# dpryan79/MethylDackel

Hardware: AMD Instinct MI355X
Metric: CpG calls/sec, synthetic 1 Mb contig 30x paired-end WGBS BAM, CpG extract (higher is better)
Workload: dtype u8/u32

## Files before the change

methyldackel_amd/csrc/mdk_prep.hip:

```cpp
#include <algorithm>
#include <atomic>
#include <mutex>
#include "mdk_hip_internal.hpp"
#include "mdk_pair_rule.h"

#ifndef PB
#define PB 256
#endif
#define MAXG 16
#define CNT_READY 0x80000000u

__device__ __forceinline__ uint32_t ld16(const uint8_t *p) { uint16_t v; __builtin_memcpy(&v, p, 2); return v; }
__device__ __forceinline__ uint32_t ld32(const uint8_t *p) { uint32_t v; __builtin_memcpy(&v, p, 4); return v; }
__device__ __forceinline__ uint64_t ld64(const uint8_t *p) { uint64_t v; __builtin_memcpy(&v, p, 8); return v; }
__device__ __forceinline__ uint4 ld128(const uint8_t *p) { uint4 v; __builtin_memcpy(&v, p, 16); return v; }

struct PrepParams {
    const uint8_t *raw; uint64_t raw_bytes; const uint32_t *rec_off; int n_rec;
    md_prep_cfg cfg; int32_t tid; int64_t beg, end, woff, wlen;
    const char *ref; int64_t reflen;
    const uint32_t *mapbits; int64_t maplen;
    const md_region *runs; int64_t nruns; int bed_on;
    PrepRead *rd; uint32_t *aidx;
    unsigned long long *hent; int32_t *hnext, *hfwd; uint32_t hmask;
// ... 430 lines not shown
#define SCAN_WAVE_LDS(NP) GW_LDS(NP)
#else
#define SCAN_WAVE_LDS(NP) RAWWIN_LDS
#endif
template <int NP>
__device__ __forceinline__ int scan_wave(const PrepParams &P, const int i, const int i0, const int lane, uint8_t *const win, PrepRead &D, uint64_t &h) {
    const RecAt at = rec_at(P, i);
#if PREP_STAGE == 2
    (void)i0;
    stage_gather<NP>(P, i, at, lane, win);
    bool far = false;
    const int adm = scan_one_gather<NP>(P, i, at, lane, win, D, h, far);
    const unsigned long long fm = __ballot(far);
    if(fm && lane == 0) atomicAdd(&P.cnt->far, (uint32_t)__popcll(fm));
    return adm;
#else
    uint32_t wbase, wlen;
    stage_window(P, i0, at, lane, win, wbase, wlen);
    return scan_one(P, i, at, win, wbase, wlen, D, h);
#endif
}
#define RDQ 3
static_assert(sizeof(PrepRead) == RDQ * sizeof(uint4), "PrepRead in quads");
__device__ __forceinline__ void stage_read(uint4 *st, const PrepRead &D, const int adm) {
    st[0] = make_uint4((uint32_t)D.pos, (uint32_t)D.rend, (uint32_t)D.ncig | (uint32_t)D.flag << 16, (uint32_t)D.strand | (uint32_t)D.nlen << 8 | (uint32_t)(adm ? 1u : 0u) << 16 | (uint32_t)D.lqn << 24);
    st[1] = make_uint4(D.name[0], D.name[1], D.name[2], D.name[3]);
    st[2] = make_uint4(D.lq, (uint32_t)D.prev, D.cig[0], D.cig[1]);
}

__device__ __forceinline__ void lds_only_barrier() { asm volatile("s_waitcnt lgkmcnt(0)\n\ts_barrier" ::: "memory"); }

__device__ __forceinline__ uint32_t static_ticket(const PrepMulti &M, int cj) {
    const uint32_t xcd = blockIdx.x & 7u, per = (7u - (uint32_t)cj) / (uint32_t)M.n + 1u;
    return (blockIdx.x >> 3) * per + xcd / (uint32_t)M.n;
}
__device__ __forceinline__ void table_insert(const PrepParams &P, int i, uint32_t sl, unsigned long long key, unsigned long long mine, unsigned long long old) {
    int32_t before = -1;
    for(;;) {
        if(old == 0ull) break;
        if((old >> 32) == (key >> 32)) {
            for(;;) { const unsigned long long seen = sync_cas(&P.hent[sl], old, mine); if(seen == old) break; old = seen; }
            before = (int32_t)(uint32_t)old - 1;
            break;
        }
        sl = (sl + 1) & P.hmask;
        old = sync_cas(&P.hent[sl], 0ull, mine);
    }
    P.hnext[i] = before;
    if(before >= 0) P.hfwd[before] = i;
}

template <int NP>
__device__ __forceinline__ void prep_scan_body(const PrepMulti &M) {
    __shared__ uint32_t wcnt[PB / 64]; __shared__ int32_t wlast[PB / 64];
    extern __shared__ __align__(16) uint4 dyn[];
    uint4 *const stage = dyn;
    const int cj = chunk_of_block(M);
    const PrepParams &P = M.P[cj];
    const uint32_t tk = static_ticket(M, cj);
    if(tk >= (uint32_t)P.nblocks) return;
    const int i = (int)(tk * PB + threadIdx.x), lane = threadIdx.x & 63, wave = threadIdx.x >> 6;
    PrepRead D; memset(&D, 0, sizeof(D)); uint64_t h = 0;
    uint8_t *const win = (uint8_t *)dyn + (size_t)wave * SCAN_WAVE_LDS(NP);
    const int adm = scan_wave<NP>(P, i, (int)(tk * PB) + 64 * wave, lane, win, D, h);
    const unsigned long long m = __ballot(adm), below = m & ((1ull << lane) - 1ull);
    const int32_t pv_wave = __shfl(D.pos, below ? 63 - __clzll((long long)below) : 0), top = __shfl(D.pos, m ? 63 - __clzll((long long)m) : 0);
    if(lane == 0) { wcnt[wave] = (uint32_t)__popcll(m); wlast[wave] = top; }
    if(P.cfg.no_pairing) {
        uint32_t v = adm ? D.lq : 0u;
#pragma unroll
        for(int d = 32; d; d >>= 1) { const uint32_t t = (uint32_t)__shfl_xor((int)v, d); v = t > v ? t : v; }
        if(lane == 0 && v) atomicMax(&P.cnt->max_lq, v);
    }
    const bool ins = adm && !P.cfg.no_pairing;
    lds_only_barrier();
    if(adm) {
        int32_t pv = pv_wave;
        if(!below) {
            pv = tk == 0 ? PREP_PREV_NONE : PREP_PREV_UNKNOWN;
            for(int w = wave - 1; w >= 0; w--) if(wcnt[w]) { pv = wlast[w]; break; }
        }
        D.prev = pv;
    }
    if(threadIdx.x == 0) {
        uint32_t t = 0; int32_t lastpos = PREP_PREV_NONE;
        for(int w = 0; w < PB / 64; w++) { t += wcnt[w]; if(wcnt[w]) lastpos = wlast[w]; }
        if(t) atomicAdd(&P.cnt->n_adm, t);
        P.cntA[tk] = (uint32_t)lastpos;
    }
    const int i0 = (int)(tk * PB);
    int32_t lprev = -2;
    uint32_t ghead = threadIdx.x;
#if PREP_LOCAL
    {
        unsigned long long *const lh = (unsigned long long *)(stage + RDQ * PB); uint32_t *const lt = (uint32_t *)(lh + PB), *const lhead = lt + 2 * PB;
        lh[threadIdx.x] = ins ? h : 0ull; lt[threadIdx.x] = 0u; lt[threadIdx.x + PB] = 0u; lhead[threadIdx.x] = 0xffffffffu;
        lds_only_barrier();
        uint32_t rep = threadIdx.x;
        if(ins) {
            uint32_t e = (uint32_t)(h >> 20) & (2u * PB - 1u);
            for(;;) {
                const uint32_t was = atomicCAS(&lt[e], 0u, threadIdx.x + 1u);
                if(was == 0u) break;
                if(lh[was - 1u] == h) { rep = was - 1u; break; }
                e = (e + 1u) & (2u * PB - 1u);
            }
            lprev = (int32_t)atomicExch(&lhead[rep], threadIdx.x);
        }
        lds_only_barrier();
        if(ins && lprev == -1) ghead = lhead[rep];
    }
#else
    if(ins) lprev = -1;
#endif
    const bool gins = ins && lprev == -1;
    const unsigned long long key = (unsigned long long)(uint32_t)(h >> 32) << 32, mine = key | (unsigned long long)((uint32_t)i0 + ghead + 1u);
    uint32_t sl = (uint32_t)h & P.hmask;
    unsigned long long old = 0ull;
#if PREP_EXP_NOCAS
    if(gins) P.hent[sl] = mine;
#else
    if(gins) old = sync_cas(&P.hent[sl], 0ull, mine);
#endif
    if(ins && lprev >= 0) { P.hnext[i] = i0 + lprev; P.hfwd[i0 + lprev] = i; }
    stage_read(stage + RDQ * threadIdx.x, D, adm);
    lds_only_barrier();
    {
        const int cnt = P.n_rec - i0 < PB ? P.n_rec - i0 : PB;
        uint4 *out = (uint4 *)(P.rd + i0);
#if !(PREP_EXP_SCAN & 1)
        for(int q = threadIdx.x; q < RDQ * cnt; q += PB) out[q] = stage[q];
#else
        if(cnt < 0) out[threadIdx.x] = stage[threadIdx.x];
#endif
    }
    if(gins) table_insert(P, i, sl, key, mine, old);
}

__global__ __launch_bounds__(PB) void k_prep_scan(const PrepMulti M) { prep_scan_body<GW_NP>(M); }
__global__ __launch_bounds__(PB) void k_prep_scan_wide(const PrepMulti M) { prep_scan_body<GW_NP_WIDE>(M); }

__global__ __launch_bounds__(PB) void k_prep_scan_ordered(const PrepMulti M) {
    constexpr int NP = GW_NP;
    __shared__ uint32_t s_tk, wcnt[PB / 64], red[PB / 64];
    extern __shared__ __align__(16) uint4 dyn[];
    uint4 *const stage = dyn;
    const PrepParams &P = M.P[chunk_of_block(M)];
    if(threadIdx.x == 0) s_tk = sync_add(&P.ticket[0], 1u);
    __syncthreads();
    const uint32_t tk = s_tk; const int i = (int)(tk * PB + threadIdx.x), lane = threadIdx.x & 63, wave = threadIdx.x >> 6;
    if(tk >= (uint32_t)P.nblocks) return;
    PrepRead D; memset(&D, 0, sizeof(D)); uint64_t h = 0;
    uint8_t *const win = (uint8_t *)dyn + (size_t)wave * SCAN_WAVE_LDS(NP);
    const int adm = scan_wave<NP>(P, i, (int)(tk * PB) + 64 * wave, lane, win, D, h);
    const unsigned long long m = __ballot(adm);
    if(lane == 0) wcnt[wave] = (uint32_t)__popcll(m);
    __syncthreads();
    uint32_t rank = (uint32_t)__popcll(m & ((1ull << lane) - 1ull)), total = 0;
    for(int w = 0; w < PB / 64; w++) { if(w < wave) rank += wcnt[w]; total += wcnt[w]; }
    if(threadIdx.x == 0) sync_set(&P.cntA[tk], total | CNT_READY);
    const uint32_t base = tickets_before(P.cntA, tk, red);
    if((int)tk == P.nblocks - 1 && threadIdx.x == 0) P.cnt->n_adm = base + total;
    if(adm) {
        if(P.aidx) P.aidx[base + rank] = (uint32_t)i;
        D.prev = PREP_PREV_UNKNOWN;
        stage_read(stage + RDQ * rank, D, 1);
    }
    __syncthreads();
    {
        uint4 *out = (uint4 *)(P.rd + base);
        for(uint32_t q = threadIdx.x; q < RDQ * total; q += PB) out[q] = stage[q];
    }
}

struct RdRegs {
    uint4 q0, q1, q2; uint32_t o;
    __device__ __forceinline__ int32_t pos() const { return (int32_t)q0.x; }
    __device__ __forceinline__ int32_t rend() const { return (int32_t)q0.y; }
    __device__ __forceinline__ uint32_t ncig() const { return q0.z & 0xffffu; }
    __device__ __forceinline__ uint32_t flag() const { return q0.z >> 16; }
    __device__ __forceinline__ uint32_t strand() const { return q0.w & 255u; }
    __device__ __forceinline__ uint32_t nlen() const { return (q0.w >> 8) & 255u; }
    __device__ __forceinline__ bool adm() const { return (q0.w >> 16) & 1u; }
    __device__ __forceinline__ uint32_t qn_off() const { return o + 36u; }
    __device__ __forceinline__ uint32_t cig_off() const { return o + 36u + (q0.w >> 24); }
    __device__ __forceinline__ uint32_t seq_off() const { return o + 36u + (q0.w >> 24) + 4u * (q0.z & 0xffffu); }
    __device__ __forceinline__ uint32_t lq() const { return q2.x; }
    __device__ __forceinline__ int32_t prev() const { return (int32_t)q2.y; }
};
__device__ __forceinline__ RdRegs rd_zero() { RdRegs R; R.q0 = R.q1 = R.q2 = make_uint4(0, 0, 0, 0); R.o = 0; return R; }
__device__ __forceinline__ RdRegs rd_load(const PrepParams &P, const uint32_t x) { const uint4 *q = (const uint4 *)&P.rd[x]; RdRegs R; R.q0 = q[0]; R.q1 = q[1]; R.q2 = q[2]; R.o = P.rec_off[P.aidx ? P.aidx[x] : x]; return R; }

struct OtherRead { int32_t rend, prev; uint32_t flag, nlen; uint4 name; };
__device__ __forceinline__ OtherRead other_read(const PrepRead *rd, const int32_t x) {
    const uint4 *q = (const uint4 *)&rd[x]; const uint4 q0 = q[0], q1 = q[1]; const uint32_t pv = ((const uint32_t *)q)[9];
    OtherRead O; O.rend = (int32_t)q0.y; O.flag = q0.z >> 16; O.nlen = (q0.w >> 8) & 255u; O.name = q1; O.prev = (int32_t)pv;
    return O;
}
__device__ __forceinline__ bool same_name(const uint8_t *raw, const uint32_t xnlen, const uint4 xname, const uint32_t xqn_off, const uint32_t ynlen, const uint4 yname, const uint32_t yqn_off) {
    if(xnlen != ynlen || xname.x != yname.x || xname.y != yname.y || xname.z != yname.z || xname.w != yname.w) return false;
    if(xnlen <= 16) return true;
    const uint8_t *p = raw + xqn_off, *q = raw + yqn_off;
    for(uint32_t k = 16; k < xnlen; k += 8) {
        uint64_t a = ld64(p + k), b = ld64(q + k);
        if(xnlen - k < 8) { const uint64_t m = (1ull << (8 * (xnlen - k))) - 1ull; a &= m; b &= m; }
        if(a != b) return false;
    }
    return true;
}
__device__ __forceinline__ int32_t block_prev(const uint32_t *last, int32_t blk, int32_t v) {
    if(blk <= 0) return PREP_PREV_NONE;
    while(v == PREP_PREV_NONE && --blk > 0) v = (int32_t)last[blk - 1];
    return v;
}
__device__ __forceinline__ int32_t prev_of(const PrepRead *rd, const int32_t x, const int32_t prev) {
    if(prev != PREP_PREV_UNKNOWN) return prev;
    for(int32_t j = (x & ~(PB - 1)) - 1; j >= 0; j--) {
        const uint4 q0 = *(const uint4 *)&rd[j];
        if((q0.w >> 16) & 1u) return (int32_t)q0.x;
    }
    return PREP_PREV_NONE;
}
#define PAIR_SECOND 0x40000000
struct PairCtx { const int32_t *hnext, *hfwd; const PrepRead *rd; const uint32_t *rec_off; const uint8_t *raw; int32_t tid; };
__device__ __forceinline__ int32_t pair_of_many(const PairCtx X, MdkPairState &S, const uint32_t a, const int32_t a_rend, const int32_t a_prev, const uint32_t a_flag, const uint32_t a_nlen, const uint4 a_name, const uint32_t a_qn_off) {
    int32_t head = (int32_t)a; int k = 0;
    for(int guard = 0; X.hfwd[head] >= 0; head = X.hfwd[head]) if(++guard > MAXG) return -2;
    for(int32_t x = head; x >= 0; x = X.hnext[x]) if(++k > MAXG) return -2;
    mdk_pair_init(S);
    for(int32_t last = -1;;) {
        int32_t x = 0x7fffffff;
        for(int32_t y = head; y >= 0; y = X.hnext[y]) if(y > last && y < x) x = y;
        if(x == 0x7fffffff) break;
        last = x;
        int32_t rend = a_rend, prev = a_prev; uint32_t flag = a_flag;
        if((uint32_t)x != a) { const OtherRead O = other_read(X.rd, x); if(!same_name(X.raw, a_nlen, a_name, a_qn_off, O.nlen, O.name, X.rec_off[x] + 36u)) continue; rend = O.rend; flag = O.flag; prev = O.prev; }
        prev = prev_of(X.rd, x, prev);
        mdk_pair_step(S, X.tid, a, x, flag, rend, prev == PREP_PREV_NONE, prev);
        if(S.overflow) return -2;
    }
    return S.mate < 0 ? -1 : (S.mate | (S.second ? PAIR_SECOND : 0));
}

struct RunIt {
    uint32_t cig_off; unsigned long long pk; int n, k; int32_t x, y, lq;
    int32_t rx, ry, rl;
    __device__ __forceinline__ bool valid() const { return rl > 0; }
    __device__ void init(const uint8_t *raw, const RdRegs &r) { cig_off = r.cig_off(); pk = (unsigned long long)r.q2.z | (unsigned long long)r.q2.w << 32; n = (int)r.ncig(); k = 0; x = r.pos(); y = 0; lq = (int32_t)r.lq(); rx = ry = rl = 0; next(raw); }
    __device__ void stop() { rl = 0; }
    __device__ void next(const uint8_t *raw) {
        rl = 0;
        while(k < n) {
            const uint32_t c = (k < 3 && (long long)pk < 0) ? (uint32_t)(pk >> (21 * k)) & 0x1fffffu : ld32(raw + cig_off + 4 * k); k++;
            const int op = c & 15; const int32_t len = (int32_t)(c >> 4);
            if(op == 0 || op == 7 || op == 8) {
                int32_t l = len; if(y + l > lq) l = lq - y;
                const int32_t sx = x, sy = y;
                x += len; y += len;
                if(l > 0) { rx = sx; ry = sy; rl = l; return; }
            } else if(op == 1 || op == 4) y += len;
            else if(op == 2 || op == 3) x += len;
        }
    }
};

struct NoSink { __device__ __forceinline__ void operator()(uint32_t, uint4, uint4) const {} };
template <bool WRITE, typename Sink>
__device__ __forceinline__ uint32_t read_segments(const PrepParams &P, const RdRegs &r, const bool has_mate, const RdRegs &m, const bool is_second, const Sink sink, const uint32_t base, const uint32_t limit, int32_t &lo, int32_t &hi) {
    const bool paired = has_mate && (((int)r.strand() - (int)m.strand()) & 1) == 0;
    RunIt own, oth;
    own.init(P.raw, r);
    if(paired) oth.init(P.raw, m); else oth.stop();
    const uint32_t sf = (r.strand() & 7) | ((r.flag() & 0x80) ? MDK_SF_READ2 : 0) | (is_second ? MDK_SF_SECOND : 0);
    const uint32_t msf = paired ? ((m.strand() & 7) | ((m.flag() & 0x80) ? MDK_SF_READ2 : 0)) : 0;
    uint32_t n = 0;
    for(; own.valid(); own.next(P.raw)) {
        int32_t cur = own.rx; const int32_t stop = own.rx + own.rl;
        while(cur < stop) {
            int32_t pe = stop; bool covered = false;
            while(oth.valid() && oth.rx + oth.rl <= cur) oth.next(P.raw);
            if(oth.valid()) { if(oth.rx <= cur) { covered = true; if(oth.rx + oth.rl < pe) pe = oth.rx + oth.rl; } else if(oth.rx < pe) pe = oth.rx; }
            if(pe - cur > 65535) pe = cur + 65535;
            if((int64_t)pe > P.beg && (int64_t)cur < P.end) {
                if(WRITE) {
                    const uint4 g0 = make_uint4((uint32_t)cur, r.seq_off(), r.lq(), (uint32_t)(own.ry + (cur - own.rx)));
                    uint4 g1 = make_uint4((uint32_t)(pe - cur) & 0xffffu | sf << 16, 0u, 0u, 0u);
                    if(covered) g1 = make_uint4((uint32_t)(pe - cur) & 0xffffu | (sf | MDK_SF_PARTNER) << 16 | msf << 24, m.seq_off(), m.lq(), (uint32_t)(oth.ry + (cur - oth.rx)));
                    const uint32_t o = base + n;
                    if(o < limit) sink(o, g0, g1);
                    if(cur < lo) lo = cur;
                    if(pe > hi) hi = pe;
                }
                n++;
            }
            cur = pe;
        }
    }
    return n;
}
static_assert(sizeof(md_seg) == 32 && offsetof(md_seg, len) == 16 && offsetof(md_seg, sf) == 18 && offsetof(md_seg, msf) == 19 && offsetof(md_seg, m_off4) == 20, "md_seg layout (read_segments builds it as two quads)");

#define SEG_STAGE 512
#define SEG_TSPAN 32
#ifndef SEGS_SGPRS
#define SEGS_SGPRS 96
#endif
#if SEGS_SGPRS
__global__ __launch_bounds__(PB, 8) __attribute__((amdgpu_num_sgpr(SEGS_SGPRS))) void k_prep_segs(const PrepMulti M) {
#else
__global__ __launch_bounds__(PB, 8) void k_prep_segs(const PrepMulti M) {
#endif
    __shared__ uint32_t s_tk, wsum[PB / 64], red[PB / 64]; __shared__ unsigned long long wbytes[PB / 64];
    __shared__ __align__(16) uint4 sstage[2 * SEG_STAGE];
    __shared__ int s_tlo, s_thi, tfirst[SEG_TSPAN], tlast[SEG_TSPAN];
    static_assert(sizeof(sstage) >= PB * sizeof(MdkPairState), "the rare path keeps a state per thread in the stage's memory");
    const PrepParams &P = M.P[chunk_of_block(M)];
#if PREP_EXP_SEGS & 8
    if(threadIdx.x == 0) s_tk = (blockIdx.x >> 3) * ((7u - (uint32_t)chunk_of_block(M)) / (uint32_t)M.n + 1u) + (blockIdx.x & 7u) / (uint32_t)M.n;
#else
    if(threadIdx.x == 0) s_tk = sync_add(&P.ticket[1], 1u);
#endif
    if(threadIdx.x == 0) { s_tlo = 0x7fffffff; s_thi = -1; }
    if(threadIdx.x < SEG_TSPAN) { tfirst[threadIdx.x] = 0x7fffffff; tlast[threadIdx.x] = 0; }
    __syncthreads();
    const uint32_t tk = s_tk, n_rec = (uint32_t)P.n_rec;
    if(tk * PB >= n_rec) return;
    const uint32_t a = tk * PB + threadIdx.x; const int lane = threadIdx.x & 63, wave = threadIdx.x >> 6;
    RdRegs r = rd_zero(), m = rd_zero(); bool has_mate = false, is_second = false; int32_t mate = -1;
    int32_t lnext = -1, lfwd = -1;
    const int32_t mylast = tk > 0 ? (int32_t)P.cntA[tk - 1] : PREP_PREV_NONE;
    if(a < n_rec) { r = rd_load(P, a); if(!P.cfg.no_pairing) { lnext = P.hnext[a]; lfwd = P.hfwd[a]; } }
    const bool active = a < n_rec && r.adm();
    uint32_t n = 0; unsigned long long bytes = 0;
    if(active) {
        if(!P.cfg.no_pairing && mdk_pairs(r.flag())) {
            const int32_t c = lnext >= 0 ? lnext : lfwd;
            if(c >= 0) {
                const int32_t cn = P.hnext[c], cf = P.hfwd[c];
                m = rd_load(P, (uint32_t)c);
                const int32_t cblk = c / PB, clast = cblk > 0 ? (int32_t)P.cntA[cblk - 1] : PREP_PREV_NONE;
                const bool more = lnext >= 0 ? (lfwd >= 0 || cn >= 0) : cf >= 0;
                const int32_t rprev = r.prev() == PREP_PREV_UNKNOWN ? block_prev(P.cntA, (int32_t)tk, mylast) : r.prev();
                const int32_t mprev = m.prev() == PREP_PREV_UNKNOWN ? block_prev(P.cntA, cblk, clast) : m.prev();
                int32_t mi = -1;
                if(!more) {
                    if(same_name(P.raw, r.nlen(), r.q1, r.qn_off(), m.nlen(), m.q1, m.qn_off())) {
                        const bool a_first = a < (uint32_t)c;
                        const int32_t f = a_first ? (int32_t)a : c, sx = a_first ? c : (int32_t)a;
                        const int32_t prev_f = a_first ? rprev : mprev, prev_s = a_first ? mprev : rprev;
                        mi = mdk_pair_two(P.tid, a, f, sx, a_first ? r.flag() : m.flag(), a_first ? r.rend() : m.rend(), prev_f == PREP_PREV_NONE, prev_f,
                                          a_first ? m.flag() : r.flag(), a_first ? m.rend() : r.rend(), prev_s, is_second);
                    }
                } else {
                    PairCtx X; X.hnext = P.hnext; X.hfwd = P.hfwd; X.rd = P.rd; X.rec_off = P.rec_off; X.raw = P.raw; X.tid = P.tid;
                    mi = pair_of_many(X, ((MdkPairState *)sstage)[threadIdx.x], a, r.rend(), r.prev(), r.flag(), r.nlen(), r.q1, r.qn_off());
                    if(mi == -2) { atomicExch(&P.cnt->fallback, 1u); mi = -1; }
                    if(mi >= 0) { is_second = (mi & PAIR_SECOND) != 0; mi &= ~PAIR_SECOND; m = rd_load(P, (uint32_t)mi); }
                }
                has_mate = mi >= 0; mate = mi;
            }
        }
        int32_t lo = 0, hi = 0;
        n = read_segments<false>(P, r, has_mate, m, is_second, NoSink(), 0u, 0u, lo, hi);
        bytes = 16ull + 4ull * r.ncig() + ((unsigned long long)r.lq() + 1) / 2 + r.lq();
    }
    uint32_t incl = n;
#pragma unroll
    for(int d = 1; d < 64; d <<= 1) { const uint32_t t = __shfl_up(incl, d); if(lane >= d) incl += t; }
    if(lane == 63) wsum[wave] = incl;
    { unsigned long long b = bytes;
#pragma unroll
      for(int d = 32; d; d >>= 1) b += __shfl_xor(b, d);
      if(lane == 0) wbytes[wave] = b; }
    __syncthreads();
    uint32_t wpos = incl - n, total = 0;
    for(int w = 0; w < PB / 64; w++) { if(w < wave) wpos += wsum[w]; total += wsum[w]; }
    if(threadIdx.x == 0) sync_set(&P.cntS[tk], total | CNT_READY);
    if(!(PREP_EXP_SEGS & 16) && threadIdx.x == 64) { unsigned long long b = 0; for(int w = 0; w < PB / 64; w++) b += wbytes[w]; if(b) atomicAdd((unsigned long long *)&P.cnt->algo_bytes, b); }
    int32_t lo = INT32_MAX, hi = INT32_MIN;
    int t0 = 0x7fffffff, t1 = -1;
    uint32_t before = 0;
    const uint32_t cap = P.cap_seg > 0xffffffffll ? 0xffffffffu : (uint32_t)P.cap_seg;
    uint4 *const st = sstage;
    if(n && !(PREP_EXP_SEGS & 2))
        (void)read_segments<true>(P, r, has_mate, m, is_second, [st](uint32_t o, uint4 g0, uint4 g1) { st[2 * o] = g0; st[2 * o + 1] = g1; }, wpos, (uint32_t)SEG_STAGE, lo, hi);
    if(n && hi > lo) {
        const int64_t l = lo < P.beg ? P.beg : (int64_t)lo, u = hi > P.end ? P.end : (int64_t)hi;
        t0 = (int)((uint32_t)(l - P.beg) / (uint32_t)P.tile); t1 = (int)((uint32_t)(u - 1 - P.beg) / (uint32_t)P.tile);
        atomicMin(&s_tlo, t0); atomicMax(&s_thi, t1);
    }
    before = (PREP_EXP_SEGS & 4) ? tk * 352u : tickets_before(P.cntS, tk, red);
    if((tk + 1) * PB >= n_rec && threadIdx.x == 0) P.cnt->n_segs = before + total;
    {
        const uint32_t left = total < SEG_STAGE ? total : SEG_STAGE;
        const uint32_t avail = cap > before ? (left < cap - before ? left : cap - before) : 0u;
        uint4 *out = (uint4 *)(P.seg + before);
        for(uint32_t q = threadIdx.x; q < 2 * avail; q += PB) out[q] = sstage[q];
    }
    if(total > SEG_STAGE && n && wpos + n > SEG_STAGE && !(PREP_EXP_SEGS & 2)) {
        const RdRegs r2 = rd_load(P, a), m2 = has_mate ? rd_load(P, (uint32_t)mate) : rd_zero();
        md_seg *const sg = P.seg + before; int32_t lo2 = 0, hi2 = 0;
        (void)read_segments<true>(P, r2, has_mate, m2, is_second, [sg](uint32_t o, uint4 g0, uint4 g1) { if(o >= SEG_STAGE) { uint4 *q = (uint4 *)(sg + o); q[0] = g0; q[1] = g1; } }, wpos, cap > before ? cap - before : 0u, lo2, hi2);
    }
    const int tlo = s_tlo, thi = s_thi;
    if(thi >= tlo && !(PREP_EXP_SEGS & 1)) {
        if(thi - tlo < SEG_TSPAN) {
            const int p0 = __shfl_up(t0, 1), p1 = __shfl_up(t1, 1), n0 = __shfl_down(t0, 1), n1 = __shfl_down(t1, 1);
            for(int t = t0; t <= t1; t++) {
                if(lane == 0 || t < p0 || t > p1) atomicMin(&tfirst[t - tlo], (int)wpos);
                if(lane == 63 || t < n0 || t > n1) atomicMax(&tlast[t - tlo], (int)(wpos + n));
            }
            __syncthreads();
            const int k = (int)threadIdx.x;
            if(k <= thi - tlo && tlast[k] > tfirst[k] && before + (uint32_t)tfirst[k] < cap) {
                const uint32_t top = before + (uint32_t)tlast[k];
                atomicMin(&P.tiles[tlo + k].first, (int)(before + (uint32_t)tfirst[k]));
                atomicMax(&P.tiles[tlo + k].last, (int)(top < cap ? top : cap));
            }
        } else {
            const uint32_t base = before + wpos; uint32_t top = base + n; if(top > cap) top = cap;
            if(base < cap) for(int t = t0; t <= t1; t++) { atomicMin(&P.tiles[t].first, (int)base); atomicMax(&P.tiles[t].last, (int)top); }
        }
    }
}

__global__ __launch_bounds__(PB) void k_perread_raw(const PrepParams P, const uint8_t *ctxcode, int64_t wend, md_pr_count *out) {
    const uint32_t a = blockIdx.x * PB + threadIdx.x;
    if(a >= P.cnt->n_adm) return;
    const RdRegs r = rd_load(P, a);
    const uint8_t *seq = P.raw + r.seq_off(), *qual = seq + ((r.lq() + 1) >> 1), *cg = P.raw + r.cig_off();
    const unsigned long long pk = (unsigned long long)r.q2.z | (unsigned long long)r.q2.w << 32;
    out[a] = perread_walk(seq, qual, r.lq(), (int)r.ncig(), r.pos(), r.strand() & 1, ctxcode, P.reflen, wend, P.cfg.min_phred, [cg, pk](int k) { return (k < 3 && (long long)pk < 0) ? (uint32_t)(pk >> (21 * k)) & 0x1fffffu : ld32(cg + 4 * k); });
}

__global__ __launch_bounds__(256) void k_rebase(uint32_t *dst, const uint32_t *src, uint32_t n, uint32_t add) {
    const uint32_t i = blockIdx.x * 256 + threadIdx.x;
    if(i < n) dst[i] = src[i] + add;
}

static int copy_ranges(md_dev *h, Slot *s, const md_raw_batch *b) {
    bool any_tab = false; uint64_t nrec_sum = 0, loose = 0;
    for(int i = 0; i < b->n_ranges; i++) { const md_raw_range &r = b->range[i]; if(r.d_rec_off || r.h_rec_off) any_tab = true; else loose += r.n_records; nrec_sum += r.n_records; }
    if((any_tab ? loose : (uint64_t)b->n_records) && !b->rec_off) return fail(MDK_ERR_ARG, "md_dev_upload_raw: null record table", hipSuccess);
    if(any_tab && nrec_sum != (uint64_t)b->n_records) return fail(MDK_ERR_ARG, "md_dev_upload_raw: with a range that has its own record table every range must carry its record count", hipSuccess);
    if(b->n_records && s->h_rectab.need((size_t)b->n_records + 1)) return MDK_ERR_NOMEM;
    uint64_t o = 0; uint32_t idx = 0, hidx = 0;
    for(int i = 0; i < b->n_ranges; i++) {
        const md_raw_range &r = b->range[i];
        if(r.d_rec_off) {
            if(r.bytes) HIPCHK(hipMemcpyAsync(s->d_raw.p + o, r.ptr, (size_t)r.bytes, hipMemcpyDeviceToDevice, s->stream));
            if(r.n_records) hipLaunchKernelGGL(k_rebase, dim3((r.n_records + 255) / 256), dim3(256), 0, s->stream, s->d_recoff.p + idx, r.d_rec_off, r.n_records, (uint32_t)o - r.rec_delta);
        } else {
            if(r.bytes) { host_block_ensure_registered(r.ptr); HIPCHK(hipMemcpyAsync(s->d_raw.p + o, r.ptr, (size_t)r.bytes, hipMemcpyHostToDevice, s->stream)); }
            if(r.h_rec_off) {
                if(r.n_records) {
                    memcpy(s->h_rectab.p + idx, r.h_rec_off, sizeof(uint32_t) * (size_t)r.n_records);
                    HIPCHK(hipMemcpyAsync(s->d_recoff.p + idx, s->h_rectab.p + idx, sizeof(uint32_t) * (size_t)r.n_records, hipMemcpyHostToDevice, s->stream));
                    hipLaunchKernelGGL(k_rebase, dim3((r.n_records + 255) / 256), dim3(256), 0, s->stream, s->d_recoff.p + idx, (const uint32_t *)(s->d_recoff.p + idx), r.n_records, (uint32_t)o - r.rec_delta);
                }
            } else {
                if(any_tab && r.n_records) {
                    memcpy(s->h_rectab.p + idx, b->rec_off + hidx, sizeof(uint32_t) * (size_t)r.n_records);
                    HIPCHK(hipMemcpyAsync(s->d_recoff.p + idx, s->h_rectab.p + idx, sizeof(uint32_t) * (size_t)r.n_records, hipMemcpyHostToDevice, s->stream));
                }
                hidx += r.n_records;
            }
        }
        idx += r.n_records; o += r.bytes;
    }
    if(!any_tab && b->n_records) {
        memcpy(s->h_rectab.p, b->rec_off, sizeof(uint32_t) * (size_t)b->n_records);
        HIPCHK(hipMemcpyAsync(s->d_recoff.p, s->h_rectab.p, sizeof(uint32_t) * (size_t)b->n_records, hipMemcpyHostToDevice, s->stream));
    }
    HIPCHK(hipGetLastError());
    return 0;
}
extern "C" int md_dev_read_raw(md_dev *h, int slot, uint8_t *bytes, uint64_t *n_bytes, uint32_t *rec_off, uint32_t *n_records) {
    Slot *s = get_slot(h, slot);
    if(!s || !s->raw_layout || !bytes || !n_bytes || !rec_off || !n_records) return fail(MDK_ERR_ARG, "md_dev_read_raw: needs a slot uploaded with md_dev_upload_raw", hipSuccess);
    if(*n_bytes < s->raw_bytes || *n_records < (uint32_t)s->pr_nrec) { *n_bytes = s->raw_bytes; *n_records = (uint32_t)s->pr_nrec; return fail(MDK_ERR_ARG, "md_dev_read_raw: buffers too small", hipSuccess); }
    HIPCHK(hipSetDevice(h->device));
    HIPCHK(hipStreamSynchronize(s->stream));
    if(s->raw_bytes) HIPCHK(hipMemcpy(bytes, s->raw_at + s->inplace_delta, (size_t)s->raw_bytes, hipMemcpyDeviceToHost));
    if(s->pr_nrec) HIPCHK(hipMemcpy(rec_off, s->rec_at, sizeof(uint32_t) * (size_t)s->pr_nrec, hipMemcpyDeviceToHost));
    if(s->inplace_delta) for(int i = 0; i < s->pr_nrec; i++) rec_off[i] -= s->inplace_delta;
    *n_bytes = s->raw_bytes; *n_records = (uint32_t)s->pr_nrec;
    return 0;
}

extern "C" int md_dev_set_prep(md_dev *h, const md_prep_cfg *cfg) {
    if(!h || !cfg) return fail(MDK_ERR_ARG, "md_dev_set_prep", hipSuccess);
    h->prep = *cfg; h->prep_set = true;
    return 0;
}

extern "C" int md_dev_set_mappability(md_dev *h, int32_t tid, const uint32_t *bits, int64_t n_bases) {
    if(!h || tid < 0 || n_bases < 0 || (n_bases && !bits)) return fail(MDK_ERR_ARG, "md_dev_set_mappability", hipSuccess);
    HIPCHK(hipSetDevice(h->device));
    if((size_t)tid >= h->mapbits.size()) { h->mapbits.resize(tid + 1, nullptr); h->maplen.resize(tid + 1, 0); }
    if(h->mapbits[tid]) { (void)hipFree(h->mapbits[tid]); h->mapbits[tid] = nullptr; h->maplen[tid] = 0; }
    const size_t words = (size_t)((n_bases + 31) / 32);
    uint32_t *d = nullptr;
    hipError_t e = hipMalloc((void **)&d, (words + 2) * 4);
    if(e != hipSuccess) return fail(MDK_ERR_NOMEM, "hipMalloc(mappability)", e);
    if(words) { e = hipMemcpy(d, bits, words * 4, hipMemcpyHostToDevice); if(e != hipSuccess) { (void)hipFree(d); return fail(MDK_ERR_HIP, "hipMemcpy(mappability)", e); } }
    h->mapbits[tid] = d; h->maplen[tid] = n_bases;
    return 0;
}

#define PREP_SCAN_LDS_MIN ((size_t)(RDQ * PB * sizeof(uint4) + PB * 8 + 2 * PB * 4 + PB * 4))
#if PREP_STAGE
#define PREP_SCAN_LDS_NP(NP) (((size_t)(PB / 64) * SCAN_WAVE_LDS(NP)) > PREP_SCAN_LDS_MIN ? ((size_t)(PB / 64) * SCAN_WAVE_LDS(NP)) : PREP_SCAN_LDS_MIN)
#else
#define PREP_SCAN_LDS_NP(NP) PREP_SCAN_LDS_MIN
#endif
#define PREP_SCAN_LDS PREP_SCAN_LDS_NP(GW_NP)
#define PREP_SCAN_LDS_WIDE PREP_SCAN_LDS_NP(GW_NP_WIDE)
static_assert(PREP_SCAN_LDS >= RDQ * PB * sizeof(uint4) + PB * 8 + 2 * PB * 4 + PB * 4, "the PrepRead stage and the workgroup's name grouping live in the windows' memory");
MDK_HIDDEN int prep_kernels_init() {
    static std::once_flag once; static int rc = 1;
    std::call_once(once, [] { rc = (hipFuncSetAttribute((const void *)k_prep_scan, hipFuncAttributeMaxDynamicSharedMemorySize, (int)PREP_SCAN_LDS) == hipSuccess &&
                                    hipFuncSetAttribute((const void *)k_prep_scan_wide, hipFuncAttributeMaxDynamicSharedMemorySize, (int)PREP_SCAN_LDS_WIDE) == hipSuccess &&
                                    hipFuncSetAttribute((const void *)k_prep_scan_ordered, hipFuncAttributeMaxDynamicSharedMemorySize, (int)PREP_SCAN_LDS) == hipSuccess) ? 0 : 1; });
    return rc;
}
static uint32_t pow2_at_least(size_t n) { uint32_t p = 1024; while(p < n) p <<= 1; return p; }

static size_t zero_bytes_for(uint32_t hmask, int nb) { return (((size_t)hmask + 1) * 8 + (size_t)(nb > 0 ? nb : 1) * 8 + 8 + 15) & ~(size_t)15; }
static void fill_prep(md_dev *h, Slot *s, PrepParams &P) {
    memset(&P, 0, sizeof(P));
    const int n = s->pr_nrec, nb = (n + PB - 1) / PB; const size_t H = (size_t)s->hmask + 1;
    P.raw = s->raw_at; P.raw_bytes = s->raw_span; P.rec_off = s->rec_at; P.n_rec = n;
    P.cfg = h->prep; P.tid = s->tid; P.beg = s->beg; P.end = s->end; P.woff = s->woff; P.wlen = s->wlen;
    P.ref = h->ref[s->tid]; P.reflen = h->reflen[s->tid];
    if(h->prep.map_on && (size_t)s->tid < h->mapbits.size()) { P.mapbits = h->mapbits[s->tid]; P.maplen = h->maplen[s->tid]; }
    P.bed_on = (size_t)s->tid < h->d_runs.size() && h->has_runs[s->tid]; if(P.bed_on) { P.runs = h->d_runs[s->tid]; P.nruns = h->n_runs[s->tid]; }
    P.rd = s->d_prd.p; P.aidx = h->prep.perread ? s->d_aidx.p : nullptr; P.hmask = s->hmask;
    const bool links = !h->prep.perread && !h->prep.no_pairing;
    P.hnext = links ? s->d_hnext.p : nullptr; P.hfwd = links ? s->d_hnext.p + (((size_t)n + 4) & ~(size_t)3) : nullptr;
    uint8_t *z = s->d_zero.p;
    P.hent = (unsigned long long *)z; P.cntA = (uint32_t *)(z + H * 8); P.cntS = P.cntA + (nb > 0 ? nb : 1); P.ticket = P.cntS + (nb > 0 ? nb : 1);
    P.nblocks = nb; P.zero = z; P.zero_bytes = zero_bytes_for(s->hmask, nb);
    P.seg = s->d_seg_in.p; P.cap_seg = (int64_t)s->d_seg_in.cap;
    P.tiles = s->d_tiles.p; P.ntiles = s->ntiles; P.tile = s->tile;
    P.cnt = s->d_pcnt.p;
}
int enqueue_prep_group(md_dev *h, Slot *const *ss, int n, hipStream_t st) {
    if(n < 1 || n > MAXM) return fail(MDK_ERR_ARG, "enqueue_prep_group", hipSuccess);
    for(int i = 0; i < n; i++) if((size_t)ss[i]->tid >= h->ref.size() || !h->ref[ss[i]->tid]) { snprintf(mdk_err_buf(), MDK_ERR_BYTES, "reference for tid %d not uploaded", ss[i]->tid); return MDK_ERR_NOREF; }
    if(prep_kernels_init()) return fail(MDK_ERR_HIP, "hipFuncSetAttribute(k_prep_scan)", hipGetLastError());
    static_assert(sizeof(PrepMulti) <= 4096, "kernel arguments are limited to 4 KiB");
    PrepMulti M; memset(&M, 0, sizeof(M));
    int total = 0; size_t zmax = 0;
    for(int i = 0; i < n; i++) { fill_prep(h, ss[i], M.P[i]); M.bstart[i] = total; total += M.P[i].nblocks; zmax = std::max<size_t>(zmax, (size_t)M.P[i].zero_bytes); ss[i]->prep_pending = false; }
    M.n = n; M.bstart[n] = total;
    int zgrid = (int)std::min<size_t>(256, (zmax / 16 + PB - 1) / PB); if(zgrid < 1) zgrid = 1;
    hipLaunchKernelGGL(k_prep_zero, dim3(zgrid * n), dim3(PB), 0, st, M);
    if(total > 0) {
        int grid = total;
        {
            int per8 = 1;
            for(int j = 0; j < n; j++) { int xcds = 0; for(int x = 0; x < 8; x++) if(x % n == j) xcds++; if(xcds) per8 = std::max(per8, (M.P[j].nblocks + xcds - 1) / xcds); else per8 = std::max(per8, M.P[j].nblocks); }
            grid = 8 * per8;
        }
        static_assert(MAXM <= 8, "chunk_of_block deals the chunks of a launch to 8 XCDs");
        if(h->prep.perread) hipLaunchKernelGGL(k_prep_scan_ordered, dim3(grid), dim3(PB), PREP_SCAN_LDS, st, M);
        else {
            if(h->scan_wide.load(std::memory_order_relaxed)) hipLaunchKernelGGL(k_prep_scan_wide, dim3(grid), dim3(PB), PREP_SCAN_LDS_WIDE, st, M);
            else hipLaunchKernelGGL(k_prep_scan, dim3(grid), dim3(PB), PREP_SCAN_LDS, st, M);
            hipLaunchKernelGGL(k_prep_segs, dim3(grid), dim3(PB), 0, st, M);
        }
    }
    HIPCHK(hipGetLastError());
    return 0;
}
static int enqueue_prep(md_dev *h, Slot *s, hipStream_t st = nullptr) { Slot *one[1] = {s}; return enqueue_prep_group(h, one, 1, st ? st : s->stream); }

static int upload_raw(md_dev *h, int slot, const md_raw_batch *b, bool may_stay) {
    Slot *s = get_slot(h, slot);
    if(!s || !b || b->n_records < 0 || b->n_ranges < 0 || b->end < b->beg) return fail(MDK_ERR_ARG, "md_dev_upload_raw", hipSuccess);
    if(!h->prep_set) return fail(MDK_ERR_ARG, "md_dev_upload_raw: md_dev_set_prep was not called", hipSuccess);
    if(b->n_records && !b->range) return fail(MDK_ERR_ARG, "md_dev_upload_raw: null array", hipSuccess);
    if(b->tid < 0) return fail(MDK_ERR_ARG, "md_dev_upload_raw: contig", hipSuccess);
    HIPCHK(hipSetDevice(h->device));
    struct SlowCall { double t0, t_sync = 0, t_alloc = 0; const md_raw_batch *b; bool on; SlowCall(const md_raw_batch *bb) : t0(mdk_prof_on() ? mdk_now() : 0), b(bb), on(mdk_prof_on()) {}
        ~SlowCall() { if(on) { const double t = mdk_now(); if(t - t0 > 0.004) { char w[256]; snprintf(w, sizeof(w), "slow upload_raw: %.1f ms (slot wait %.1f, buffers %.1f, copies %.1f), %d ranges, %d records, first range %s", (t - t0) * 1e3, (t_sync - t0) * 1e3, (t_alloc - t_sync) * 1e3, (t - t_alloc) * 1e3, b->n_ranges, b->n_records, b->n_ranges ? (b->range[0].d_rec_off ? "device" : b->range[0].h_rec_off ? "host+table" : "host") : "-"); mdk_marks_dump(w); } } } } slow(b);
    if(s->busy) {
        ProfScope pf(PF_UP_SYNC);
        HIPCHK(hipStreamSynchronize(s->stream));
        if(s->run && s->run != s->stream) HIPCHK(hipStreamSynchronize(s->run));
    }
    slow.t_sync = slow.on ? mdk_now() : 0;
    s->busy = true;
    s->fresh = true;
    uint64_t total = 0;
    for(int i = 0; i < b->n_ranges; i++) total += b->range[i].bytes;
    if(total >= (1ull << 32) - 64) return fail(MDK_ERR_ARG, "md_dev_upload_raw: more than 4 GiB of records in one chunk", hipSuccess);
    const int64_t span = b->end - b->beg; const int TILE = h->tile;
    const int ntiles = (int)((span + TILE - 1) / TILE), n = b->n_records, nb = (n + PB - 1) / PB;
    s->tid = b->tid; s->beg = b->beg; s->end = b->end; s->woff = b->woff; s->wlen = b->wlen; s->uploaded = false; s->launched = false;
    s->tile = TILE; s->ntiles = ntiles; s->lds_bytes = TILE * ((h->variant ? 16 : 8) + 4);
    s->pr_nrec = n; s->raw_bytes = total; s->raw_layout = true; s->n_segs = -1; s->n_reads = -1; s->read_bytes = 0;
    static const bool no_inplace = getenv("MDK_NO_INPLACE") != nullptr;
    const bool inplace = may_stay && !no_inplace && b->n_ranges == 1 && b->range[0].d_rec_off && (uint32_t)n == b->range[0].n_records && n > 0 && b->range[0].bytes + (uint64_t)b->range[0].rec_delta < (1ull << 32) - 64;
    const size_t nn = (size_t)n + 1, nt = (size_t)(ntiles > 0 ? ntiles : 1);
    const size_t segcap = std::max<size_t>(s->d_seg_in.cap, nn * 2 + 4096);
    s->hmask = pow2_at_least(nn + nn / 4) - 1;
    static std::atomic<int> first_call{1}; const bool first = mdk_prof_on() && first_call.exchange(0); const double tf0 = first ? mdk_now() : 0; double tf1 = 0;
    {
        ProfScope pf(PF_UP_ALLOC);
        if((!inplace && (s->d_raw.need((size_t)total + 64) || s->d_recoff.need(nn))) || s->d_prd.need(nn) || s->d_hnext.need(2 * nn + 8) || s->d_zero.need(zero_bytes_for(s->hmask, nb)) ||
           s->d_seg_in.need(segcap) || s->d_tiles.need(nt) || s->d_seg.need(nt)) return MDK_ERR_NOMEM;
        if(!s->b_site) {
            if(s->d_site.need((size_t)span + 16)) return MDK_ERR_NOMEM;
            if(h->variant && s->d_var.need((size_t)span + 16)) return MDK_ERR_NOMEM;
        }
    }
    if(first) tf1 = mdk_now();
    slow.t_alloc = slow.on ? mdk_now() : 0;
    if(inplace) { const md_raw_range &r = b->range[0]; s->inplace = true; s->inplace_delta = r.rec_delta; s->raw_at = r.ptr - r.rec_delta; s->rec_at = r.d_rec_off; s->raw_span = (uint64_t)r.rec_delta + r.bytes; HIPCHK(hipEventRecord(s->e1, s->stream)); }
    else { ProfScope pf(PF_UP_COPY); s->inplace = false; s->inplace_delta = 0; s->raw_at = s->d_raw.p; s->rec_at = s->d_recoff.p; s->raw_span = total; int rcc = copy_ranges(h, s, b); if(rcc) return rcc; HIPCHK(hipEventRecord(s->e1, s->stream)); }
    if(first) fprintf(stderr, "[mdk hip] the first chunk's upload: device buffers %.3fs, registration + copies queued %.3fs\n", tf1 - tf0, mdk_now() - tf1);
    s->prep_pending = true;
    s->uploaded = true;
    return inplace ? 1 : 0;
}
extern "C" int md_dev_upload_raw(md_dev *h, int slot, const md_raw_batch *b) { return upload_raw(h, slot, b, false); }
extern "C" int md_dev_upload_raw_inplace(md_dev *h, int slot, const md_raw_batch *b) { return upload_raw(h, slot, b, true); }

extern "C" int md_dev_upload_wait(md_dev *h, int slot) {
    Slot *s = get_slot(h, slot);
    if(!s || !s->uploaded) return fail(MDK_ERR_ARG, "md_dev_upload_wait: slot not uploaded", hipSuccess);
    HIPCHK(hipSetDevice(h->device));
    if(s->raw_layout) HIPCHK(hipEventSynchronize(s->e1)); else HIPCHK(hipStreamSynchronize(s->stream));
    return 0;
}

extern "C" int md_dev_upload_done(md_dev *h, int slot) {
    Slot *s = get_slot(h, slot);
    if(!s || !s->uploaded) return fail(MDK_ERR_ARG, "md_dev_upload_done: slot not uploaded", hipSuccess);
    HIPCHK(hipSetDevice(h->device));
    const hipError_t e = s->raw_layout ? hipEventQuery(s->e1) : hipStreamQuery(s->stream);
    if(e == hipSuccess) return 1;
    if(e == hipErrorNotReady) { (void)hipGetLastError(); return 0; }
    return fail(MDK_ERR_HIP, "hipEventQuery", e);
}

extern "C" int md_dev_submit_raw(md_dev *h, int slot, const md_raw_batch *b) {
    int rc = md_dev_upload_raw(h, slot, b);
    if(rc) return rc;
    return md_dev_launch(h, slot);
}

extern "C" int md_dev_perread_submit_raw(md_dev *h, int slot, const md_raw_batch *b) {
    Slot *s = get_slot(h, slot);
    if(!s || !b || b->n_records < 0 || b->n_ranges < 0 || b->end < b->beg) return fail(MDK_ERR_ARG, "md_dev_perread_submit_raw", hipSuccess);
    if(!h->prep_set || !h->prep.perread) return fail(MDK_ERR_ARG, "md_dev_perread_submit_raw: md_dev_set_prep with perread first", hipSuccess);
    if(b->n_records && !b->range) return fail(MDK_ERR_ARG, "md_dev_perread_submit_raw: null array", hipSuccess);
    if(b->tid < 0 || (size_t)b->tid >= h->ref.size() || !h->ref[b->tid]) { snprintf(mdk_err_buf(), MDK_ERR_BYTES, "reference for tid %d not uploaded", b->tid); return MDK_ERR_NOREF; }
    HIPCHK(hipSetDevice(h->device));
    HIPCHK(hipStreamSynchronize(s->stream));
    s->busy = true;
    s->pr_n = -1; s->uploaded = false; s->launched = false;
// ... 104 lines not shown
```

Measured before the change: 6.883 billion.

## Stage block's reads plus halo in LDS for mate lookups in k_prep_segs

```diff
diff --git a/methyldackel_amd/csrc/mdk_prep.hip b/methyldackel_amd/csrc/mdk_prep.hip
--- a/methyldackel_amd/csrc/mdk_prep.hip
+++ b/methyldackel_amd/csrc/mdk_prep.hip
@@ -756,6 +756,13 @@
 
 #define SEG_STAGE 512
 #define SEG_TSPAN 32
+#ifndef SEGS_HALO
+#define SEGS_HALO 32
+#endif
+static_assert(SEGS_HALO >= 0 && SEGS_HALO <= PB, "k_prep_segs: a read in the window lies in the workgroup's block or a neighbour of it");
+#define SEGS_WIN (PB + 2 * SEGS_HALO)
+#define SEGS_WIN_QUADS ((SEGS_WIN * (RDQ * 16 + 12) + 15) / 16)
+#define SEGS_LDS_QUADS (SEGS_WIN_QUADS > 2 * SEG_STAGE ? SEGS_WIN_QUADS : 2 * SEG_STAGE)
 #ifndef SEGS_SGPRS
 #define SEGS_SGPRS 96
 #endif
@@ -765,9 +772,11 @@
 __global__ __launch_bounds__(PB, 8) void k_prep_segs(const PrepMulti M) {
 #endif
     __shared__ uint32_t s_tk, wsum[PB / 64], red[PB / 64]; __shared__ unsigned long long wbytes[PB / 64];
-    __shared__ __align__(16) uint4 sstage[2 * SEG_STAGE];
+    __shared__ __align__(16) uint4 sstage[SEGS_LDS_QUADS];
+    __shared__ int32_t s_last[3];
     __shared__ int s_tlo, s_thi, tfirst[SEG_TSPAN], tlast[SEG_TSPAN];
     static_assert(sizeof(sstage) >= PB * sizeof(MdkPairState), "the rare path keeps a state per thread in the stage's memory");
+    static_assert(sizeof(sstage) >= 2 * SEG_STAGE * sizeof(uint4), "the segment stage lives in the same memory");
     const PrepParams &P = M.P[chunk_of_block(M)];
 #if PREP_EXP_SEGS & 8
     if(threadIdx.x == 0) s_tk = (blockIdx.x >> 3) * ((7u - (uint32_t)chunk_of_block(M)) / (uint32_t)M.n + 1u) + (blockIdx.x & 7u) / (uint32_t)M.n;
@@ -782,37 +791,82 @@
     const uint32_t a = tk * PB + threadIdx.x; const int lane = threadIdx.x & 63, wave = threadIdx.x >> 6;
     RdRegs r = rd_zero(), m = rd_zero(); bool has_mate = false, is_second = false; int32_t mate = -1;
     int32_t lnext = -1, lfwd = -1;
-    const int32_t mylast = tk > 0 ? (int32_t)P.cntA[tk - 1] : PREP_PREV_NONE;
-    if(a < n_rec) { r = rd_load(P, a); if(!P.cfg.no_pairing) { lnext = P.hnext[a]; lfwd = P.hfwd[a]; } }
+    const bool pairing = !P.cfg.no_pairing;
+    const uint32_t i0 = tk * PB, halo = pairing ? (uint32_t)SEGS_HALO : 0u;
+    const uint32_t w0 = i0 > halo ? i0 - halo : 0u, w1 = i0 + PB + halo < n_rec ? i0 + PB + halo : n_rec, wn = w1 - w0;
+    uint4 *const wq = sstage; uint32_t *const woff = (uint32_t *)(sstage + RDQ * SEGS_WIN); int32_t *const wnext = (int32_t *)woff + SEGS_WIN, *const wfwd = wnext + SEGS_WIN;
+    {
+        constexpr int NQ = (RDQ * SEGS_WIN + PB - 1) / PB, NR = (SEGS_WIN + PB - 1) / PB;
+        const uint4 *const src = (const uint4 *)(P.rd + w0);
+        uint4 vq[NQ]; uint32_t vo[NR]; int32_t vn[NR], vf[NR], vl = PREP_PREV_NONE;
+#pragma unroll
+        for(int k = 0; k < NQ; k++) { const uint32_t q = threadIdx.x + (uint32_t)k * PB; vq[k] = src[q < RDQ * wn ? q : RDQ * wn - 1u]; }
+#pragma unroll
+        for(int k = 0; k < NR; k++) { const uint32_t j = threadIdx.x + (uint32_t)k * PB; vo[k] = P.rec_off[w0 + (j < wn ? j : wn - 1u)]; }
+        if(pairing) {
+#pragma unroll
+            for(int k = 0; k < NR; k++) { const uint32_t j = threadIdx.x + (uint32_t)k * PB, x = w0 + (j < wn ? j : wn - 1u); vn[k] = P.hnext[x]; vf[k] = P.hfwd[x]; }
+        } else {
+#pragma unroll
+            for(int k = 0; k < NR; k++) vn[k] = vf[k] = -1;
+        }
+        const uint32_t lk = threadIdx.x < 3 ? threadIdx.x : 2u;
+        { const int32_t b = (int32_t)tk - 2 + (int32_t)lk; vl = (int32_t)P.cntA[b >= 0 ? b : 0]; if(b < 0) vl = PREP_PREV_NONE; }
+#pragma unroll
+        for(int k = 0; k < NQ; k++) { const uint32_t q = threadIdx.x + (uint32_t)k * PB; wq[q < RDQ * wn ? q : RDQ * wn - 1u] = vq[k]; }
+#pragma unroll
+        for(int k = 0; k < NR; k++) { const uint32_t j = threadIdx.x + (uint32_t)k * PB, jc = j < wn ? j : wn - 1u; woff[jc] = vo[k]; wnext[jc] = vn[k]; wfwd[jc] = vf[k]; }
+        s_last[lk] = vl;
+    }
+    __syncthreads();
+    int32_t c = -1, cn = -1, cf = -1, clast = PREP_PREV_NONE; bool far = false;
+    if(a < n_rec) {
+        const uint32_t j = a - w0;
+        r.q0 = wq[RDQ * j]; r.q1 = wq[RDQ * j + 1]; r.q2 = wq[RDQ * j + 2]; r.o = woff[j];
+        lnext = wnext[j]; lfwd = wfwd[j];
+    }
     const bool active = a < n_rec && r.adm();
+    if(active && pairing && mdk_pairs(r.flag())) {
+        c = lnext >= 0 ? lnext : lfwd;
+        if(c >= 0) {
+            if((uint32_t)c >= w0 && (uint32_t)c < w1) {
+                const uint32_t j = (uint32_t)c - w0;
+                m.q0 = wq[RDQ * j]; m.q1 = wq[RDQ * j + 1]; m.q2 = wq[RDQ * j + 2]; m.o = woff[j];
+                cn = wnext[j]; cf = wfwd[j];
+                clast = s_last[c / PB - (int32_t)tk + 1];
+            } else far = true;
+        }
+    }
+    const int32_t mylast = s_last[1];
+    lds_only_barrier();
+    if(far) {
+        cn = P.hnext[c]; cf = P.hfwd[c];
+        m = rd_load(P, (uint32_t)c);
+        const int32_t cblk = c / PB; clast = cblk > 0 ? (int32_t)P.cntA[cblk - 1] : PREP_PREV_NONE;
+    }
     uint32_t n = 0; unsigned long long bytes = 0;
     if(active) {
-        if(!P.cfg.no_pairing && mdk_pairs(r.flag())) {
-            const int32_t c = lnext >= 0 ? lnext : lfwd;
-            if(c >= 0) {
-                const int32_t cn = P.hnext[c], cf = P.hfwd[c];
-                m = rd_load(P, (uint32_t)c);
-                const int32_t cblk = c / PB, clast = cblk > 0 ? (int32_t)P.cntA[cblk - 1] : PREP_PREV_NONE;
-                const bool more = lnext >= 0 ? (lfwd >= 0 || cn >= 0) : cf >= 0;
-                const int32_t rprev = r.prev() == PREP_PREV_UNKNOWN ? block_prev(P.cntA, (int32_t)tk, mylast) : r.prev();
-                const int32_t mprev = m.prev() == PREP_PREV_UNKNOWN ? block_prev(P.cntA, cblk, clast) : m.prev();
-                int32_t mi = -1;
-                if(!more) {
-                    if(same_name(P.raw, r.nlen(), r.q1, r.qn_off(), m.nlen(), m.q1, m.qn_off())) {
-                        const bool a_first = a < (uint32_t)c;
-                        const int32_t f = a_first ? (int32_t)a : c, sx = a_first ? c : (int32_t)a;
-                        const int32_t prev_f = a_first ? rprev : mprev, prev_s = a_first ? mprev : rprev;
-                        mi = mdk_pair_two(P.tid, a, f, sx, a_first ? r.flag() : m.flag(), a_first ? r.rend() : m.rend(), prev_f == PREP_PREV_NONE, prev_f,
-                                          a_first ? m.flag() : r.flag(), a_first ? m.rend() : r.rend(), prev_s, is_second);
-                    }
-                } else {
-                    PairCtx X; X.hnext = P.hnext; X.hfwd = P.hfwd; X.rd = P.rd; X.rec_off = P.rec_off; X.raw = P.raw; X.tid = P.tid;
-                    mi = pair_of_many(X, ((MdkPairState *)sstage)[threadIdx.x], a, r.rend(), r.prev(), r.flag(), r.nlen(), r.q1, r.qn_off());
-                    if(mi == -2) { atomicExch(&P.cnt->fallback, 1u); mi = -1; }
-                    if(mi >= 0) { is_second = (mi & PAIR_SECOND) != 0; mi &= ~PAIR_SECOND; m = rd_load(P, (uint32_t)mi); }
+        if(c >= 0) {
+            const int32_t cblk = c / PB;
+            const bool more = lnext >= 0 ? (lfwd >= 0 || cn >= 0) : cf >= 0;
+            const int32_t rprev = r.prev() == PREP_PREV_UNKNOWN ? block_prev(P.cntA, (int32_t)tk, mylast) : r.prev();
+            const int32_t mprev = m.prev() == PREP_PREV_UNKNOWN ? block_prev(P.cntA, cblk, clast) : m.prev();
+            int32_t mi = -1;
+            if(!more) {
+                if(same_name(P.raw, r.nlen(), r.q1, r.qn_off(), m.nlen(), m.q1, m.qn_off())) {
+                    const bool a_first = a < (uint32_t)c;
+                    const int32_t f = a_first ? (int32_t)a : c, sx = a_first ? c : (int32_t)a;
+                    const int32_t prev_f = a_first ? rprev : mprev, prev_s = a_first ? mprev : rprev;
+                    mi = mdk_pair_two(P.tid, a, f, sx, a_first ? r.flag() : m.flag(), a_first ? r.rend() : m.rend(), prev_f == PREP_PREV_NONE, prev_f,
+                                      a_first ? m.flag() : r.flag(), a_first ? m.rend() : r.rend(), prev_s, is_second);
                 }
-                has_mate = mi >= 0; mate = mi;
+            } else {
+                PairCtx X; X.hnext = P.hnext; X.hfwd = P.hfwd; X.rd = P.rd; X.rec_off = P.rec_off; X.raw = P.raw; X.tid = P.tid;
+                mi = pair_of_many(X, ((MdkPairState *)sstage)[threadIdx.x], a, r.rend(), r.prev(), r.flag(), r.nlen(), r.q1, r.qn_off());
+                if(mi == -2) { atomicExch(&P.cnt->fallback, 1u); mi = -1; }
+                if(mi >= 0) { is_second = (mi & PAIR_SECOND) != 0; mi &= ~PAIR_SECOND; m = rd_load(P, (uint32_t)mi); }
             }
+            has_mate = mi >= 0; mate = mi;
         }
         int32_t lo = 0, hi = 0;
         n = read_segments<false>(P, r, has_mate, m, is_second, NoSink(), 0u, 0u, lo, hi);
```

Measured after the change: 6.864 billion. Within noise of the previous version (-0.3%).
